# david-andrew/TerminalRayTracer

Hardware: AMD Instinct MI355X
Metric: path rays/s (primary+secondary) at 1920x1080, 64 spheres, 8 bounces (higher is better)
Workload: dtype f64

## Files before the change

include/trt_hip_diag.h:

```cpp
#ifndef TRT_HIP_DIAG_H
#define TRT_HIP_DIAG_H

#include "trt_hip.h"

#ifdef __cplusplus
extern "C" {
#endif

int trt_set_list_pool_words(trt_context *ctx, size_t words);

int trt_enable_counters(trt_context *ctx, int enable);

int trt_read_counters(trt_context *ctx, unsigned long long *path_rays, unsigned long long *shadow_rays);

int trt_read_diagnostics(trt_context *ctx, unsigned long long *wave_loop_trips, unsigned long long *phase2_rounds);

int trt_path_family_code(trt_context *ctx, int kind, int sphere, const double *parent_origin);

long trt_read_path_tables(trt_context *ctx, const Camera *camera, unsigned long long *cells, size_t capacity_cells,
                          unsigned long long *pool, size_t capacity_pool, long info[8]);

int trt_read_sweep_fallbacks(trt_context *ctx, unsigned long long *swept_traces);

int trt_read_shading_passes(trt_context *ctx, unsigned long long *passes);

int trt_read_loop_diagnostics(trt_context *ctx, unsigned long long out[8]);

long trt_read_light_grid(trt_context *ctx, int point_light, int index, unsigned long long *masks, size_t capacity_words);

long trt_read_light_lists(trt_context *ctx, int point_light, int index, unsigned long long *cells, size_t capacity_cells,
                          unsigned long long *pool, size_t capacity_pool, long info[4]);

int trt_selftest_div_sqrt(trt_context *ctx, const double *a, const double *b, size_t n, double *quot, double *root);

int trt_selftest_unit(trt_context *ctx, const double *xyzw, size_t n, double *fast, double *reference);

int trt_selftest_cube(trt_context *ctx, const float *xyz, size_t n, float *device_out, float *host_out);

int trt_selftest_sky(trt_context *ctx, const double *dirs, size_t n, int dim, long long *exact, long long *estimate, int *ambiguous);

int trt_probe_rays(trt_context *ctx, const Ray *rays, size_t n, int *obj, double *point, double *normal,
                   double *material, double *lit);

int trt_probe_rays_production(trt_context *ctx, const Camera *camera, const Ray *rays, const int *families, size_t n, int *obj,
                              double *point, double *normal, double *material, double *lit);

long trt_launch_count(trt_context *ctx);
int trt_launch_span_ms(trt_context *first, long first_launch, trt_context *last, long last_launch, float *ms);

int trt_set_scene_image(trt_context *ctx, int mode);

int trt_render_image(trt_context *ctx, int *in_device_memory, unsigned long long *image_bytes);

// ... 16 lines not shown
```

terminalraytracer_amd/csrc/trt_context.hpp:

```cpp
#pragma once

#include "trt_hip.h"
#include "trt_hip_diag.h"

#include <hip/hip_runtime.h>

#include <math.h>
#include <stdarg.h>
#include <stdio.h>
#include <stdlib.h>
#include <string.h>

#include <algorithm>
#include <chrono>
#include <memory>
#include <mutex>
#include <thread>
#include <vector>

#ifndef TRT_DIRGRID_CELLS
#define TRT_DIRGRID_CELLS 128
#endif
#ifndef TRT_POINTGRID_CELLS
#define TRT_POINTGRID_CELLS 64
// ... 57 lines not shown
    double m = fmod(t, 2 * kPi);
    return (m < kPi) ? (m / kPi) : (2 - (m / kPi));
}

}

using trt_impl::DeviceBuffer;
using trt_impl::Event;
using trt_impl::PinnedBuffer;
using trt_impl::Stream;
using trt_impl::kEventRing;

constexpr int kEyeSlots = 8;

struct SceneTables
{
    int device = 0;
    DeviceBuffer<double> d_spheres, d_dir, d_point;
    DeviceBuffer<float> d_cull;
    DeviceBuffer<unsigned long long> d_dir_masks, d_point_masks;
    DeviceBuffer<trt_dirgrid> d_dirgrids;
    DeviceBuffer<trt_pointgrid> d_pointgrids;
    DeviceBuffer<trt_dirgrid_disc> d_discs;
    DeviceBuffer<trt_pointgrid_cone> d_cones;
    DeviceBuffer<unsigned long long> d_dir_lists, d_point_lists, d_path_lists, d_pool;
    DeviceBuffer<unsigned long long> d_pool_used;
    DeviceBuffer<trt_rayfamily> d_families;
    DeviceBuffer<double> d_sphere_fam;
    DeviceBuffer<double> d_patch_rec;
    DeviceBuffer<uint32_t> d_sky;
    int path_built_for[4] = {-1, -1, -1, -2};
    int grids_built_for[4] = {-1, -1, -1, -1};
    size_t pool_scene_words = 0, pool_eye_words = 0;
    trt_cull_scene cull_scene{};
    double ground_built[6] = {0.0, 0.0, 0.0, 0.0, 0.0, 0.0};
    std::vector<double> h_spheres, h_dir, h_point;
    unsigned eye_slots_taken = 0;
    bool built_for_moving_scene = false;
    double build_seconds = 0.0;
    ~SceneTables() { (void)hipSetDevice(device); }
};

struct trt_context
{
    int device = 0;
    Stream own_stream;
    hipStream_t stream = nullptr;
    int compute_units = 0;
    int reserved_cus = 0;
    int lds_limit = 0;

    bool have_scene = false;
    std::shared_ptr<SceneTables> T;
    int eye_slot = 0;
    trt::SceneView scene{};
    trt::CullView cull{};
    DeviceBuffer<double> d_jitter, d_fb, d_axes, d_samples, d_samples_alt;
    DeviceBuffer<double> d_image, d_image_alt;
    trt::GridView grids{};
    int dirgrid_cells = TRT_DIRGRID_CELLS, pointgrid_cells = TRT_POINTGRID_CELLS;
    int dirgrid_slabs = TRT_DIRGRID_SLABS, pointgrid_shells = TRT_POINTGRID_SHELLS;
    int path_g_eye = TRT_PATHGRID_EYE, path_g_sph = TRT_PATHGRID_SPHERE;
    int path_min_spheres = TRT_PATHGRID_MIN_SPHERES;
    int path_patches = TRT_PATHGRID_PATCHES;
    size_t list_pool_cap = 0;
    int scene_changes_in_a_row = 0, scene_still_calls = 0;
// ... 139 lines not shown
```

terminalraytracer_amd/csrc/trt_diag.hip:

```cpp
#define TRT_UNIT_DIAG 1
#include "trt_context.hpp"
#include "trt_simple.hpp"

using namespace trt_impl;

namespace trt_impl
{
void allow_large_lds_diag(const trt_context *ctx)
{
    (void)hipFuncSetAttribute((const void *)trt::probe_rays_kernel, hipFuncAttributeMaxDynamicSharedMemorySize, ctx->lds_limit);
    (void)hipFuncSetAttribute((const void *)trt::probe_rounds_kernel<false>, hipFuncAttributeMaxDynamicSharedMemorySize, ctx->lds_limit);
    (void)hipFuncSetAttribute((const void *)trt::probe_rounds_kernel<true>, hipFuncAttributeMaxDynamicSharedMemorySize, ctx->lds_limit);
}
}

extern "C" int trt_set_list_pool_words(trt_context *ctx, size_t words)
{
    if (!ctx)
        return fail(TRT_ERR_ARGUMENT, "ctx is NULL");
    const int rc = refuse_if_shared(ctx, "trt_set_list_pool_words");
    if (rc)
        return rc;
    ctx->list_pool_cap = words;
    ctx->T->grids_built_for[0] = -1;
// ... 54 lines not shown
    const int k = trt_patch_of(ctx->grids.patch_m, parent_origin[0] - c[0], parent_origin[1] - c[1], parent_origin[2] - c[2]);
    return 2 + n + ((sphere << TRT_PATCH_SHIFT) | k);
}

extern "C" long trt_read_path_tables(trt_context *ctx, const Camera *camera, unsigned long long *cells, size_t capacity_cells,
                                     unsigned long long *pool, size_t capacity_pool, long info[8])
{
    if (!ctx || !camera || !cells || !pool || !info)
        return fail(TRT_ERR_ARGUMENT, "NULL argument");
    if (!ctx->have_scene)
        return fail(TRT_ERR_NO_SCENE, "no scene");
    HIP_TRY(hipSetDevice(ctx->device));
    const int rc = ensure_eye_tables(ctx, camera, ctx->stream);
    if (rc)
        return rc;
    HIP_TRY(hipStreamSynchronize(ctx->stream));
    const trt::GridView &g = ctx->grids;
    const int n = (int)(ctx->T->h_spheres.size() / 9);
    unsigned long long used[16 * (1 + kEyeSlots)] = {0};
    HIP_TRY(hipMemcpy(used, ctx->T->d_pool_used.ptr, sizeof used, hipMemcpyDeviceToHost));
    const size_t eye_total = 2 * 6 * (size_t)g.g_eye * g.g_eye, sph_total = 2 * (size_t)n * (size_t)g.patch_count * 6 * (size_t)g.g_sph * g.g_sph;
    const size_t total = g.path_enabled ? eye_total + sph_total : 0;
    const size_t pool_words = ctx->T->pool_scene_words + kEyeSlots * ctx->T->pool_eye_words;
    const size_t eye_from = ctx->T->pool_scene_words + (size_t)ctx->eye_slot * ctx->T->pool_eye_words;
    info[0] = g.path_enabled, info[1] = g.g_eye, info[2] = g.g_sph, info[3] = n, info[4] = (long)total;
    info[5] = (long)std::min<unsigned long long>(used[0], 1ull << 62), info[6] = (long)used[16 * (1 + ctx->eye_slot)] - (long)eye_from, info[7] = (long)pool_words;
    if (!g.path_enabled)
        return 0;
    if (capacity_cells < total || capacity_pool < pool_words)
        return fail(TRT_ERR_CAPACITY, "tables have %zu cells and %zu pool words", total, pool_words);
    HIP_TRY(hipMemcpy(cells, ctx->T->d_path_lists.ptr + g.eye_at, eye_total * sizeof(unsigned long long), hipMemcpyDeviceToHost));
    if (sph_total)
        HIP_TRY(hipMemcpy(cells + eye_total, ctx->T->d_path_lists.ptr + g.sph_at, sph_total * sizeof(unsigned long long), hipMemcpyDeviceToHost));
    HIP_TRY(hipMemcpy(pool, ctx->T->d_pool.ptr, pool_words * sizeof(unsigned long long), hipMemcpyDeviceToHost));
    return (long)total;
}

extern "C" long trt_read_light_grid(trt_context *ctx, int point_light, int index, unsigned long long *masks, size_t capacity_words)
{
    if (!ctx || !masks || index < 0)
        return fail(TRT_ERR_ARGUMENT, "bad argument");
    if (!ctx->have_scene)
        return fail(TRT_ERR_NO_SCENE, "no scene");
    const trt::GridView &g = ctx->grids;
    if (!g.enabled)
        return 0;
    if (index >= (point_light ? ctx->scene.num_point : ctx->scene.num_dir))
        return fail(TRT_ERR_ARGUMENT, "light %d", index);
    const size_t words = (size_t)std::max((ctx->scene.num_spheres + 63) / 64, 1);
    const size_t stride = (point_light ? g.point_stride : g.dir_stride) * words;
    if (capacity_words < stride)
        return fail(TRT_ERR_CAPACITY, "table has %zu words, buffer %zu", stride, capacity_words);
    HIP_TRY(hipSetDevice(ctx->device));
    HIP_TRY(hipStreamSynchronize(ctx->stream));
    HIP_TRY(hipMemcpy(masks, (point_light ? ctx->T->d_point_masks.ptr : ctx->T->d_dir_masks.ptr) + stride * (size_t)index, stride * sizeof(unsigned long long),
                      hipMemcpyDeviceToHost));
    return (long)stride;
}

extern "C" long trt_read_light_lists(trt_context *ctx, int point_light, int index, unsigned long long *cells, size_t capacity_cells,
                                     unsigned long long *pool, size_t capacity_pool, long info[4])
{
    const bool query = !cells && !pool && !capacity_cells && !capacity_pool;
    if (!ctx || !info || index < 0 || (!query && (!cells || !pool)))
        return fail(TRT_ERR_ARGUMENT, "bad argument");
    if (!ctx->have_scene)
// ... 223 lines not shown
```

terminalraytracer_amd/csrc/trt_rounds.hpp:

```cpp
#pragma once

#include "trt_device.hpp"
#include "trt_filter.h"
#include "trt_lightgrid.h"
#include "trt_raygrid.h"
#include "trt_common.hpp"

#define TRT_EXPECT_LIST(c) __builtin_expect(!!(c), 1)
#define TRT_EXPECT_RARE(c) __builtin_expect(!!(c), 0)

namespace trt
{


#define CONSTANT_AS __attribute__((address_space(4)))
template <class T>
TRT_DEV T load_kernel_argument(const char CONSTANT_AS *at)
{
    static_assert(sizeof(T) % 8 == 0 && alignof(T) == 8, "argument structs are whole 64-bit words");
    T out;
    const unsigned long long CONSTANT_AS *src = (const unsigned long long CONSTANT_AS *)at;
    unsigned long long *dst = (unsigned long long *)&out;
#pragma unroll
    for (size_t i = 0; i < sizeof(T) / 8; i++)
        dst[i] = src[i];
    return out;
}

struct GridView
{
    const trt_dirgrid *dir;
    const trt_pointgrid *point;
    const unsigned long long *dir_lists, *point_lists;
    unsigned dir_stride, point_stride;
    int enabled;
    int list_bits;
    int path_enabled;
    int g_eye, g_sph;
    int patch_m, patch_count;
    unsigned eye_at, sph_at;
    const unsigned long long *path_lists;
    const unsigned long long *pool;
    const double *sphere_fam;
    const double *patch_rec;
    double rg2_sph;
    double slack0;
    trt_rayfamily eye[2];
};

static_assert(sizeof(trt_rayfamily) == 8 * TRT_RAYFAMILY_DOUBLES, "families of the eye in the LDS image");
static_assert(sizeof(trt_dirgrid) == 8 * kDirGridDoubles && sizeof(trt_pointgrid) == 8 * kPointGridDoubles, "light-table headers in the LDS image");

constexpr int kDirRecord = 8;

struct LdsImage
{
    const float4 *cull;
    const float4 *cull_dir;
    const double *sph;
    const double *mat;
    const double *dir;
    const double *pt;
    const double *b255;
    const double *cam;
    const double *jit;
    const trt_dirgrid *dirgrid;
    const trt_pointgrid *pointgrid;
    const double *fam;
    const double *eye;
    const double *patch;
};

inline size_t rounds_lds_bytes(const SceneView &s, int spp, int patches, int frames = 1)
// ... 373 lines not shown
        k++;
        const double2 c01 = ((const double2 *)L.sph)[2 * i], c23 = ((const double2 *)L.sph)[2 * i + 1];
        const d3 oc = sub(o, d3{c01.x, c01.y, c23.x});
        const double b = 2.0 * dot(oc, d);
        const double cc = dot(oc, oc) - c23.y;
        const double disc = b * b - 4.0 * a * cc;
        if (valid && !(disc < 0.0) && b < 0.0)
        {
            const double q = -b - sqrt_exact(disc), qq = q * q;
            const bool blocks = q > TRT_SHADOW_QMIN && qq * TRT_SHADOW_K1 <= lo;
            unsure = unsure || (q > 0.0 && !blocks && !(qq >= hi));
            dark = dark || blocks;
            count = blocks ? 0 : count;
        }
    }
    {
        const double denom = dot(d, gn), num = dot(sub(gp, o), gn);
        const bool steep = __builtin_fabs(denom) > 0.00001;
        const bool same_sign = (long long)(__builtin_bit_cast(unsigned long long, num) ^ __builtin_bit_cast(unsigned long long, denom)) >= 0;
        const bool maybe = active && !dark && steep && same_sign;
        if (__any(maybe))
        {
            const double t = num / denom;
            const bool hit = maybe && t > 0.00001;
            const double qq = (t * t) * (4.0 * a) * a;
            const bool blocks = hit && qq * TRT_SHADOW_K1 <= lo;
            dark = dark || blocks;
            unsure = unsure || (hit && !blocks && !(qq >= hi));
        }
    }
    unsure = unsure && !dark;
}

template <bool BATCH = false>
TRT_DEV unsigned long long path_cell(const LdsImage &L, const GridView &G, int n, int fam, d3 o, d3 d, bool active, unsigned long long active_lanes,
                                     unsigned long long &fallback_lanes, int frame = 0)
{
    const bool in_family = fam >= 0;
    const unsigned long long family_lanes = lanes_with(in_family);
    const bool has = active && in_family;
    const int f = has ? fam : 0;
    const int s = f >= 2 ? f - 2 : 0, i = s >= n ? s - n : s;
    const bool of_eye = f < 2, mirrored = s >= n;
    const double *rec = L.fam + 4 * i;
    d3 apex = mirrored ? load3(rec) : load3(L.sph + 4 * i);
    double r_chk = mirrored ? rec[3] + TRT_FAMILY_SLACK : rec[3];
    const double *E = BATCH ? L.eye + frame * (2 * TRT_RAYFAMILY_DOUBLES) + TRT_RAYFAMILY_DOUBLES * (f & 1) : L.eye + TRT_RAYFAMILY_DOUBLES * (f & 1);
    const double rg2_eye = E[5];
    if (of_eye)
    {
        apex = load3(E);
        r_chk = E[3];
    }
    const double rg2 = of_eye ? rg2_eye : G.rg2_sph;
    const d3 w = sub(o, apex);
    const d3 c = d3{w.y * d.z - w.z * d.y, w.z * d.x - w.x * d.z, w.x * d.y - w.y * d.x};
    const bool near_line = dot(c, c) <= r_chk * r_chk, ahead = dot(w, d) >= -r_chk, in_range = dot(w, w) <= rg2;
    const bool unit_dir = __builtin_fabs(dot(d, d) - 1.0) <= 9.094947017729282e-13;
    const bool member = near_line & ahead & in_range & unit_dir;
    const unsigned long long member_lanes = family_lanes & lanes_with(near_line) & lanes_with(ahead) & lanes_with(in_range) & lanes_with(unit_dir);
    const int g = of_eye ? G.g_eye : G.g_sph;
    const int at = trt_cubemap_cell((float)d.x, (float)d.y, (float)d.z, 0.5f * (float)g, (float)(g - 1), g);
    const unsigned eye_cells = 6u * (unsigned)G.g_eye * (unsigned)G.g_eye, sph_cells = 6u * (unsigned)G.g_sph * (unsigned)G.g_sph;
    const unsigned base = of_eye ? G.eye_at + (BATCH ? 2u * (unsigned)frame + (unsigned)f : (unsigned)f) * eye_cells : G.sph_at + (unsigned)s * sph_cells;
    unsigned long long cell = 0;
    if (has && member)
        cell = G.path_lists[base + (unsigned)at];
    fallback_lanes = active_lanes & (~member_lanes | lanes_with((unsigned)(cell >> 56) == TRT_LIST_NONE));
    return cell;
}

template <bool BATCH = false>
TRT_DEV unsigned long long path_cell_patches(const LdsImage &L, const GridView &G, int n, int &fam, d3 o, d3 d, bool active, unsigned long long active_lanes,
                                             unsigned long long &fallback_lanes, int frame = 0)
{
    const bool in_family = fam >= 0;
    const unsigned long long family_lanes = lanes_with(in_family);
    const bool has = active && in_family;
    const int f = has ? fam : 0;
    const bool of_eye = f < 2, mirrored = f >= 2 + n;
    const int code = f - 2 - n;
    const int i = mirrored ? code >> TRT_PATCH_SHIFT : (of_eye ? 0 : f - 2);
    const double *at_sphere = L.sph + 4 * i, *at_mirror = L.fam + 4 * i;
    const double *src = of_eye ? L.eye + (BATCH ? frame * (2 * TRT_RAYFAMILY_DOUBLES) : 0) + TRT_RAYFAMILY_DOUBLES * (f & 1) : (mirrored ? at_mirror : at_sphere);
    const d3 base_at = load3(src);
    const int here = trt_cubemap_cell((float)(o.x - base_at.x), (float)(o.y - base_at.y), (float)(o.z - base_at.z), 0.5f * (float)G.patch_m,
                                      (float)(G.patch_m - 1), G.patch_m);
    const int k = mirrored ? code & ((1 << TRT_PATCH_SHIFT) - 1) : (of_eye ? 0 : here);
    fam = !has ? -1 : (f == 0 ? 1 : (!of_eye && !mirrored ? 2 + n + (((f - 2) << TRT_PATCH_SHIFT) | k) : -1));
    const double r_abs = of_eye ? 0.0 : at_mirror[3];
    const double *pr = L.patch + TRT_PATCH_RECORD * k + (mirrored ? 4 : 0);
    const d3 apex = d3{TRT_PATCH_APEX(base_at.x, r_abs, pr[0]), TRT_PATCH_APEX(base_at.y, r_abs, pr[1]), TRT_PATCH_APEX(base_at.z, r_abs, pr[2])};
    const double rho = pr[3];
    double rchk_eye = src[3], rg2_eye = src[5];
    asm("" : "+v"(rchk_eye), "+v"(rg2_eye));
    double r_chk = TRT_PATCH_RCHK(r_abs, rho, G.slack0), rg2 = G.rg2_sph;
    r_chk = mirrored ? r_chk + TRT_FAMILY_SLACK : r_chk;
// ... 23 lines not shown
}

struct Tally
{
    unsigned path = 0, shadow = 0, rounds = 0, swept = 0, passes = 0;
    unsigned iters[3] = {0, 0, 0};
    unsigned tests[3] = {0, 0, 0};
    unsigned full = 0;
};

struct PathHit
{
    Hit ph;
    bool hit;
    bool sky;
    unsigned long long hit_lanes, sky_lanes;
    d3 back;
    d3 normal;
    int mat;
};

template <bool COUNT, bool REFRACT = false, bool PATCHES = false, bool BATCH = false>
TRT_DEV PathHit path_stage(const LdsImage &L, const CullView &cull, const GridView &grids, int n, d3 o, d3 d, int &fam, bool alive, unsigned long long alive_lanes,
                           d3 gp, d3 gn, Tally &tally, int inside = -1, int frame = 0)
{
    bool p_list = false;
    unsigned long long p_cell = 0;
    if (grids.path_enabled)
    {
        unsigned long long fallback_lanes;
        if constexpr (PATCHES)
            p_cell = path_cell_patches<BATCH>(L, grids, n, fam, o, d, alive, alive_lanes, fallback_lanes, frame);
        else
            p_cell = path_cell<BATCH>(L, grids, n, fam, o, d, alive, alive_lanes, fallback_lanes, frame);
        p_list = fallback_lanes == 0;
    }
    if (COUNT && !p_list)
        tally.swept++;
    PathHit r;
    r.ph = trace<false, REFRACT, 2>(L, cull, n, o, d, alive, alive_lanes, gp, gn, tally.iters[0], tally.tests[0], nullptr, p_list, p_cell, grids.pool, grids.list_bits, inside);
    r.hit = alive && r.ph.i >= 0;
    r.sky = alive && r.ph.i < 0;
    r.hit_lanes = alive_lanes & lanes_with(r.ph.i >= 0);
    r.sky_lanes = alive_lanes & ~r.hit_lanes;
    if (r.hit)
        fam = r.ph.i < n ? 2 + r.ph.i : (PATCHES ? fam : (fam == 0 ? 1 : (fam >= 2 && fam < 2 + n ? fam + n : -1)));
    r.back = unit(r.hit ? sub(o, r.ph.p) : d);
    r.normal = d;
    r.mat = 0;
    if (r.hit_lanes != 0)
    {
        d3 raw = gn;
        r.mat = n + checker_odd(r.ph.p);
        if (r.ph.i >= 0 && r.ph.i < n)
        {
            raw = sub(r.ph.p, load3(L.sph + 4 * r.ph.i));
            r.mat = r.ph.i;
        }
        r.normal = unit(raw);
    }
    TRT_MARK_AT(6);
    return r;
}

template <bool COUNT>
TRT_DEV d3 shadow_stage(const LdsImage &L, const CullView &cull, const GridView &grids, int n, int nd, int nl, d3 o, d3 normal, int mat,
                        bool lit_lanes, unsigned long long lit_word, d3 gp, d3 gn, Tally &tally)
// ... 669 lines not shown
```

terminalraytracer_amd/csrc/trt_tables.hip:

```cpp
#include "trt_context.hpp"

using namespace trt_impl;

namespace
{

__global__ void build_dirgrid_kernel(const trt_dirgrid_disc *discs, int n, int g, int slabs, int words, unsigned long long *masks)
{
    const long cell = (long)blockIdx.x * blockDim.x + threadIdx.x;
    if (cell >= (long)slabs * g * g)
        return;
    const int c = (int)(cell % g), j = (int)((cell / g) % g), slab = (int)(cell / ((long)g * g));
    for (int w = 0; w < words; w++)
    {
        unsigned long long m = 0;
        for (int b = 0; b < 64 && w * 64 + b < n; b++)
            if (trt_dirgrid_in_slab(discs + w * 64 + b, slab) && trt_dirgrid_reaches(discs + w * 64 + b, c, j))
                m |= 0x8000000000000000ull >> b;
        masks[cell * words + w] = m;
    }
}

__global__ void build_pointgrid_kernel(const trt_pointgrid_cone *cones, int n, int g, int shells, int words, unsigned long long *masks)
{
// ... 10 lines not shown
        masks[cell * words + w] = m;
    }
}

__device__ unsigned long long pack_cell(const unsigned long long *mask, int words, unsigned long long *pool, unsigned long long *pool_used,
                                        unsigned pool_limit, int bits, bool valid = true)
{
    const int count = valid ? trt_list_count(mask, words) : 0;
    const unsigned need = valid ? trt_list_pool_words(count, bits) : 0u;
    const int lane = (int)(threadIdx.x & 63);
    unsigned upto = need;
#pragma unroll
    for (int d = 1; d < 64; d <<= 1)
    {
        const unsigned below = __shfl_up(upto, d);
        upto += lane >= d ? below : 0u;
    }
    const unsigned total = __shfl(upto, 63);
    unsigned long long base = 0;
    if (total)
    {
        if (lane == 63)
            base = atomicAdd(pool_used, (unsigned long long)total);
        base = __shfl(base, 63);
    }
    if (!valid)
        return 0ull;
    if (need == 0)
        return trt_list_pack(mask, words, count, nullptr, 0u, bits);
    const unsigned long long at = base + (upto - need);
    if (count > 0xffff || at + need > (unsigned long long)pool_limit)
        return (unsigned long long)TRT_LIST_NONE << 56;
    return trt_list_pack(mask, words, count, pool, (unsigned)at, bits);
}

__global__ void set_pool_counter_kernel(unsigned long long *counter, unsigned long long value) { *counter = value; }

__global__ void pack_lists_kernel(const unsigned long long *masks, long cells, int words, unsigned long long *lists, unsigned long long *pool,
                                  unsigned long long *pool_used, unsigned pool_limit, int bits)
{
    const long cell = (long)blockIdx.x * blockDim.x + threadIdx.x;
    const bool valid = cell < cells;
    const unsigned long long packed = pack_cell(masks + (valid ? cell : 0) * words, words, pool, pool_used, pool_limit, bits, valid);
    if (valid)
        lists[cell] = packed;
}

static_assert(TRT_FAMILY_TILE * TRT_FAMILY_TILE == 64, "a tile per wave");
constexpr int kSceneTilesPerBlock = 16;
unsigned family_grid_blocks(int g, int tiles_per_block)
{
    const unsigned cells = 6u * (unsigned)g * (unsigned)g;
    return trt_family_tiled(g) ? (cells / 64u + (unsigned)tiles_per_block - 1u) / (unsigned)tiles_per_block : (cells + 255u) / 256u;
}

template <int kWords>
constexpr size_t family_lds_bytes()
{
    return sizeof(trt_pointgrid_cone) * 64 * kWords + sizeof(unsigned long long) * kWords + sizeof(unsigned long long) * 4 * 64 * kWords;
}

template <int kWords>
__global__ __launch_bounds__(256) void build_family_lists_kernel(const double *spheres, int n, const trt_rayfamily *families, trt_rayfamily f0,
                                                                 trt_rayfamily f1, int by_value, int g, unsigned long long *lists,
                                                                 unsigned long long *pool, unsigned long long *pool_used, unsigned pool_limit,
                                                                 int tiles_per_block)
// ... 175 lines not shown
{
    if (ctx->path_patches >= 0)
        return std::min(ctx->path_patches, TRT_PATCH_MAX_M);
    if (ctx->moving_scene)
        return 0;
    int m = n >= TRT_PATCHES_FROM_SPHERES ? 2 : 0;
    const unsigned long long per_table = 6ull * (unsigned long long)ctx->path_g_sph * (unsigned long long)ctx->path_g_sph;
    while (m > 0 && 2ull * (unsigned long long)n * (6ull * m * m) * per_table * 12ull > kAutoPatchBudgetBytes)
        m--;
    return m;
}

static int build_path_tables(trt_context *ctx, const trt_cull_scene &cs, const double *ground)
{
    const int n = (int)(ctx->T->h_spheres.size() / 9);
    trt::GridView &g = ctx->grids;
    g.path_enabled = 0;
    g.patch_m = g.patch_count = 0;
    invalidate_eye_tables(ctx);
    ctx->T->path_built_for[0] = ctx->path_g_eye;
    ctx->T->path_built_for[1] = ctx->path_g_sph;
    ctx->T->path_built_for[2] = ctx->path_min_spheres;
    ctx->T->path_built_for[3] = ctx->path_patches;
    ctx->T->cull_scene = cs;
    memcpy(ctx->T->ground_built, ground, sizeof ctx->T->ground_built);
    const int ge = ctx->path_g_eye, gs = ctx->path_g_sph;
    if (ge < 2 || gs < 2 || n > TRT_PATH_MAX_SPHERES || n < ctx->path_min_spheres)
        return TRT_OK;
    trt_patchset patches;
    trt_patchset_init(&patches, patches_for(ctx, n));
    const size_t P = (size_t)patches.count, families = 2 * (size_t)n * P;
    const size_t eye_cells = 6 * (size_t)ge * ge, sph_cells = 6 * (size_t)gs * gs;
    const size_t eye_part = (size_t)kEyeSlots * 2 * eye_cells;
    if (eye_part + families * sph_cells >= 0xffffffffull)
        return fail(TRT_ERR_CAPACITY, "path tables of %zu families x %zu cells", families, sph_cells);
    HIP_TRY(ctx->T->d_path_lists.reserve(eye_part + families * sph_cells));
    HIP_TRY(hipMemsetAsync(ctx->T->d_path_lists.ptr, 0xFF, (eye_part + families * sph_cells) * sizeof(unsigned long long), ctx->stream));
    HIP_TRY(ctx->T->d_families.reserve(std::max<size_t>(families, 1)));
    HIP_TRY(ctx->T->d_sphere_fam.reserve(4 * (size_t)std::max(n, 1)));
    HIP_TRY(ctx->T->d_patch_rec.reserve(P * TRT_PATCH_RECORD));
    std::vector<trt_rayfamily> fam(std::max<size_t>(families, 1));
    std::vector<double> rec(4 * (size_t)std::max(n, 1)), prec(P * TRT_PATCH_RECORD);
    trt_family_consts consts;
    trt_sphere_families(ctx->T->h_spheres.data(), n, ground, &cs, &patches, fam.data(), rec.data(), &consts);
    trt_patch_records(&patches, ground, prec.data());
    HIP_TRY(hipMemcpy(ctx->T->d_patch_rec.ptr, prec.data(), prec.size() * sizeof(double), hipMemcpyHostToDevice));
    if (n)
    {
        HIP_TRY(hipMemcpy(ctx->T->d_families.ptr, fam.data(), families * sizeof(trt_rayfamily), hipMemcpyHostToDevice));
        HIP_TRY(hipMemcpy(ctx->T->d_sphere_fam.ptr, rec.data(), 4 * (size_t)n * sizeof(double), hipMemcpyHostToDevice));
        for (size_t first = 0; first < families; first += 32768)
        {
            const unsigned batch = (unsigned)std::min<size_t>(32768, families - first);
            launch_family_builder(n, dim3(family_grid_blocks(gs, kSceneTilesPerBlock), batch), ctx->stream, (const double *)ctx->T->d_spheres.ptr,
                                  (const trt_rayfamily *)ctx->T->d_families.ptr + first, trt_rayfamily{}, trt_rayfamily{}, 0, gs,
                                  ctx->T->d_path_lists.ptr + eye_part + first * sph_cells, ctx->T->d_pool.ptr, ctx->T->d_pool_used.ptr, (unsigned)ctx->T->pool_scene_words,
                                  kSceneTilesPerBlock);
        }
        HIP_TRY(hipGetLastError());
        HIP_TRY(hipStreamSynchronize(ctx->stream));
    }
    g.path_lists = ctx->T->d_path_lists.ptr;
    g.eye_at = (unsigned)((size_t)ctx->eye_slot * 2 * eye_cells);
    g.sph_at = (unsigned)eye_part;
    g.pool = ctx->T->d_pool.ptr;
    g.sphere_fam = ctx->T->d_sphere_fam.ptr;
    g.patch_rec = ctx->T->d_patch_rec.ptr;
    g.patch_m = patches.m;
    g.patch_count = patches.count;
    g.rg2_sph = consts.rg * consts.rg;
    g.slack0 = consts.slack;
    g.g_eye = ge;
    g.g_sph = gs;
    g.path_enabled = 1;
    return TRT_OK;
}

int build_tables(trt_context *ctx, const trt_cull_scene &cs, const double *ground)
{
    ctx->table_builds++;
    const size_t n = ctx->T->h_spheres.size() / 9, nd = ctx->T->h_dir.size() / 6, np = ctx->T->h_point.size() / 7;
    const size_t gd = (size_t)ctx->dirgrid_cells, gp = (size_t)ctx->pointgrid_cells, ge = (size_t)ctx->path_g_eye, gs = (size_t)ctx->path_g_sph;
    const size_t sd = (size_t)std::max(ctx->dirgrid_slabs, 1), sp = (size_t)std::max(ctx->pointgrid_shells, 1);
    const int m = patches_for(ctx, (int)n);
    const size_t sphere_cells = 2 * n * (m ? 6 * (size_t)m * m : 1) * 6 * gs * gs;
    const size_t wide = n > TRT_LIST_MAX_SPHERES ? 2 : 1, sphere_part = n > TRT_PATH_MAX_SPHERES ? 0 : (m ? sphere_cells / 2 : sphere_cells);
    ctx->T->pool_scene_words = std::max<size_t>(1024, wide * (nd * sd * gd * gd + np * 6 * sp * gp * gp + sphere_part));
    const size_t per_word = wide == 2 ? 4 : 8;
    ctx->T->pool_eye_words = std::max<size_t>(1024, 2 * 6 * ge * ge * std::min<size_t>((n + per_word - 1) / per_word, 64));
    if (ctx->list_pool_cap)
    {
        ctx->T->pool_scene_words = std::min(ctx->T->pool_scene_words, std::max<size_t>(ctx->list_pool_cap, 1));
        ctx->T->pool_eye_words = std::min(ctx->T->pool_eye_words, std::max<size_t>(ctx->list_pool_cap, 1));
    }
    const double t0 = host_seconds();
    int rc = TRT_OK;
    for (int pass = 0; pass < 2 && !rc; pass++)
    {
        if (ctx->T->pool_scene_words + kEyeSlots * ctx->T->pool_eye_words >= 0xffffffffull)
            return fail(TRT_ERR_CAPACITY, "candidate tables too large");
        ctx->grids = trt::GridView{};
        ctx->grids.list_bits = n > TRT_LIST_MAX_SPHERES ? 16 : 8;
        HIP_TRY(ctx->T->d_pool.reserve(ctx->T->pool_scene_words + kEyeSlots * ctx->T->pool_eye_words));
        HIP_TRY(ctx->T->d_pool_used.reserve(16 * (1 + kEyeSlots)));
        HIP_TRY(hipMemsetAsync(ctx->T->d_pool_used.ptr, 0, 16 * (1 + kEyeSlots) * sizeof(unsigned long long), ctx->stream));
        rc = build_light_grids(ctx, cs);
        if (!rc)
            rc = build_path_tables(ctx, cs, ground);
        if (rc || ctx->list_pool_cap)
            break;
        unsigned long long asked = 0;
        HIP_TRY(hipMemcpyAsync(&asked, ctx->T->d_pool_used.ptr, sizeof asked, hipMemcpyDeviceToHost, ctx->stream));
        HIP_TRY(hipStreamSynchronize(ctx->stream));
        if (asked <= ctx->T->pool_scene_words)
            break;
        ctx->T->pool_scene_words = (size_t)asked + 1024;
    }
    ctx->T->build_seconds = host_seconds() - t0;
    return rc;
}

static int build_eye_slot(trt_context *ctx, const trt_rayfamily *families, int slot, hipStream_t stream)
{
    const trt::GridView &g = ctx->grids;
    const int n = (int)(ctx->T->h_spheres.size() / 9), ge = g.g_eye;
    const size_t eye_cells = 6 * (size_t)ge * ge;
    const size_t pool_from = ctx->T->pool_scene_words + (size_t)slot * ctx->T->pool_eye_words;
    unsigned long long *const counter = ctx->T->d_pool_used.ptr + 16 * (1 + slot);
    hipLaunchKernelGGL(set_pool_counter_kernel, dim3(1), dim3(1), 0, stream, counter, (unsigned long long)pool_from);
    launch_family_builder(n, dim3(family_grid_blocks(ge, 1), 2u), stream, (const double *)ctx->T->d_spheres.ptr, (const trt_rayfamily *)nullptr, families[0], families[1], 1,
                          ge, ctx->T->d_path_lists.ptr + (size_t)slot * 2 * eye_cells, ctx->T->d_pool.ptr, counter, (unsigned)(pool_from + ctx->T->pool_eye_words), 1);
    HIP_TRY(hipGetLastError());
    return TRT_OK;
}

int ensure_eye_tables(trt_context *ctx, const Camera *camera, hipStream_t stream, int slot)
{
    trt::GridView &g = ctx->grids;
    if (!g.path_enabled)
        return TRT_OK;
    if (slot < 0)
        slot = ctx->eye_slot;
    trt_context::EyeSlot &built = ctx->eye_slots[slot];
    const double eye[3] = {camera->frame.origin.x, camera->frame.origin.y, camera->frame.origin.z};
    if (built.valid && !memcmp(eye, built.eye, sizeof eye))
        return TRT_OK;
    built.valid = false;
    trt_eye_families(eye, ctx->T->ground_built, &ctx->T->cull_scene, built.families);
    if (slot == ctx->eye_slot)
// ... 11 lines not shown
```

terminalraytracer_amd/hip.py:

```python
import ctypes as C
import functools
import os

import numpy as np

from . import layout as L

_HERE = os.path.dirname(os.path.abspath(__file__))
LIB_PATH = os.environ.get("TRT_HIP_LIB") or os.path.join(_HERE, "libtrt_hip.so")

TRT_OK = 0
ERRORS = {-1: "TRT_ERR_HIP", -2: "TRT_ERR_ARGUMENT", -3: "TRT_ERR_NO_SCENE", -4: "TRT_ERR_CAPACITY",
          -5: "TRT_ERR_NOT_INITIALISED"}


class TrtError(RuntimeError):
    def __init__(self, code, message):
        super().__init__(f"{ERRORS.get(code, code)}: {message}")
        self.code = code


class RowSet(C.Structure):
    _fields_ = [("width", C.c_int), ("height", C.c_int), ("tile_rows", C.c_int), ("tile_first", C.c_int),
                ("tile_step", C.c_int)]
# ... 51 lines not shown
    "trt_render_host_batch": (_I, [_VP, _VP, _I, C.POINTER(RowSet), _I, _I, _VP]),
    "trt_render_device_batch_rgb8": (_I, [_VP, _VP, _I, C.POINTER(RowSet), _I, _I, _VP, _SZ]),
    "trt_render_host_batch_rgb8": (_I, [_VP, _VP, _I, C.POINTER(RowSet), _I, _I, _VP]),
    "trt_render_device_batch_ansi": (_I, [_VP, _VP, _I, C.POINTER(RowSet), _I, _I, _VP, _SZ]),
    "trt_render_host_batch_ansi": (_I, [_VP, _VP, _I, C.POINTER(RowSet), _I, _I, _VP]),
    "trt_batch_info": (_I, [_VP, C.POINTER(_I), C.POINTER(_I)]),
    "trt_synchronize": (_I, [_VP]),
    "trt_kernel_times": (_I, [_VP, C.POINTER(C.c_float), _I]),
    "trt_render_kernel_times": (_I, [_VP, C.POINTER(C.c_float), C.POINTER(C.c_float), _I]),
    "trt_enable_counters": (_I, [_VP, _I]),
    "trt_read_counters": (_I, [_VP, C.POINTER(C.c_ulonglong), C.POINTER(C.c_ulonglong)]),
    "trt_read_diagnostics": (_I, [_VP, C.POINTER(C.c_ulonglong), C.POINTER(C.c_ulonglong)]),
    "trt_set_kernel": (_I, [_VP, _I]),
    "trt_set_light_grids": (_I, [_VP, _I, _I]),
    "trt_set_light_slabs": (_I, [_VP, _I, _I]),
    "trt_share_scene": (_I, [_VP, _VP]),
    "trt_set_scene_policy": (_I, [_I, _I]),
    "trt_scene_is_moving": (_I, []),
    "trt_scene_info": (_I, [_VP, C.POINTER(C.c_ulonglong), C.POINTER(_I), C.POINTER(C.c_double)]),
    "trt_set_list_pool_words": (_I, [_VP, C.c_size_t]),
    "trt_set_path_grids": (_I, [_VP, _I, _I]),
    "trt_set_path_grids_min_spheres": (_I, [_VP, _I]),
    "trt_set_path_patches": (_I, [_VP, _I]),
    "trt_get_path_patches": (_I, [_VP, C.POINTER(_I), C.POINTER(_I)]),
    "trt_path_family_code": (_I, [_VP, _I, _I, _VP]),
    "trt_set_compaction": (_I, [_VP, _I]),
    "trt_render_variant": (_I, [_VP, C.POINTER(_I), C.POINTER(_I)]),
    "trt_set_scene_image": (_I, [_VP, _I]),
    "trt_render_image": (_I, [_VP, C.POINTER(_I), C.POINTER(C.c_ulonglong)]),
    "trt_set_scratch_fill": (_I, [_VP, _I]),
    "trt_default_context": (_VP, []),
    "trt_build_counts": (_I, [_VP, C.POINTER(C.c_ulonglong), C.POINTER(C.c_ulonglong)]),
    "trt_read_path_tables": (C.c_long, [_VP, C.POINTER(L.Camera), _VP, C.c_size_t, _VP, C.c_size_t, C.POINTER(C.c_long)]),
    "trt_read_sweep_fallbacks": (_I, [_VP, C.POINTER(C.c_ulonglong)]),
    "trt_read_shading_passes": (_I, [_VP, C.POINTER(C.c_ulonglong)]),
    "trt_read_loop_diagnostics": (_I, [_VP, C.POINTER(C.c_ulonglong)]),
    "trt_set_refraction": (_I, [_VP, _VP, _I]),
    "trt_reserve_cus": (_I, [_VP, _I]),
    "trt_get_stream": (_I, [_VP, C.POINTER(C.c_void_p)]),
    "trt_selftest_cube": (_I, [_VP, _VP, C.c_size_t, _VP, _VP]),
    "trt_selftest_unit": (_I, [_VP, _VP, C.c_size_t, _VP, _VP]),
    "trt_selftest_sky": (_I, [_VP, _VP, C.c_size_t, _I, _VP, _VP, _VP]),
    "trt_read_light_grid": (C.c_long, [_VP, _I, _I, _VP, C.c_size_t]),
    "trt_read_light_lists": (C.c_long, [_VP, _I, _I, _VP, C.c_size_t, _VP, C.c_size_t, C.POINTER(C.c_long)]),
    "trt_kernel_info": (_I, [_VP] + [C.POINTER(_I)] * 5),
    "trt_selftest_div_sqrt": (_I, [_VP, _VP, _VP, _SZ, _VP, _VP]),
    "trt_probe_rays": (_I, [_VP, _VP, _SZ, _VP, _VP, _VP, _VP, _VP]),
    "trt_probe_rays_production": (_I, [_VP, C.POINTER(L.Camera), _VP, _VP, _SZ, _VP, _VP, _VP, _VP, _VP]),
    "trt_launch_count": (C.c_long, [_VP]),
    "trt_launch_span_ms": (_I, [_VP, C.c_long, _VP, C.c_long, C.POINTER(C.c_float)]),
    "trt_dist_unique_id": (_I, [_VP]),
    "trt_dist_frame_times": (_I, [_VP, C.POINTER(C.c_float), C.POINTER(C.c_float)]),
    "trt_dist_allow_rccl_override": (_I, [_I]),
    "trt_dist_rccl_library": (C.c_char_p, []),
    "trt_dist_comm_ranks": (_I, [_VP]),
    "trt_dist_create": (_I, [_I, C.POINTER(L.Scene), _VP, _I, _I, _I, _I, _I, _I, _I, C.POINTER(_VP)]),
    "trt_dist_set_scene": (_I, [_VP, C.POINTER(L.Scene)]),
    "trt_dist_render": (_I, [_VP, C.POINTER(L.Camera), _I, _I, C.POINTER(_VP)]),
    "trt_dist_synchronize": (_I, [_VP]),
    "trt_dist_enable_rgb8": (_I, [_VP]),
    "trt_dist_render_rgb8": (_I, [_VP, C.POINTER(L.Camera), _I, _I, C.POINTER(_VP)]),
    "trt_dist_fetch_rgb8": (_I, [_VP, _VP, _VP]),
    "trt_dist_fetch": (_I, [_VP, _VP, _VP]),
    "trt_dist_source_rows": (_I, [_I, _I, _I, _I, C.POINTER(_I)]),
    "trt_dist_info": (_I, [_VP] + [C.POINTER(_I)] * 5),
    "trt_dist_context": (_VP, [_VP, _I]),
# ... 131 lines not shown
        d, t = _I(), _I()
        _check(lib().trt_render_variant(self._h, C.byref(d), C.byref(t)))
        return {"decoupled": bool(d.value), "workgroup_threads": t.value}

    def set_scene_image(self, mode):
        _check(lib().trt_set_scene_image(self._h, mode))

    def render_image(self):
        d, b = _I(), C.c_ulonglong()
        _check(lib().trt_render_image(self._h, C.byref(d), C.byref(b)))
        return {"in_device_memory": bool(d.value), "image_bytes": b.value}

    def build_counts(self):
        b, u = C.c_ulonglong(), C.c_ulonglong()
        _check(lib().trt_build_counts(self._h, C.byref(b), C.byref(u)))
        return b.value, u.value

    def set_scratch_fill(self, on=True):
        _check(lib().trt_set_scratch_fill(self._h, 1 if on else 0))

    def read_path_tables(self, camera_array):
        cam = camera_struct(camera_array)
        info = (C.c_long * 8)()
        probe = np.zeros(1, dtype=np.uint64)
        lib().trt_read_path_tables(self._h, C.byref(cam), probe.ctypes.data, 0, probe.ctypes.data, 0, info)
        cells = np.zeros(max(1, info[4]), dtype=np.uint64)
        pool = np.zeros(max(1, info[7]), dtype=np.uint64)
        got = lib().trt_read_path_tables(self._h, C.byref(cam), cells.ctypes.data, cells.size, pool.ctypes.data, pool.size, info)
        if got < 0:
            _check(int(got))
        keys = ("enabled", "eye_cells", "sphere_cells", "spheres", "cells", "pool_used_scene", "pool_used_eye", "pool_capacity")
        return dict(zip(keys, [int(x) for x in info])), cells[:got], pool

    def set_refraction(self, ior=None):
        if ior is None:
            _check(lib().trt_set_refraction(self._h, None, 0))
        else:
            a = np.ascontiguousarray(ior, dtype=np.float64)
            _check(lib().trt_set_refraction(self._h, a.ctypes.data, a.size))

    def read_sweep_fallbacks(self):
        v = C.c_ulonglong()
        _check(lib().trt_read_sweep_fallbacks(self._h, C.byref(v)))
        return v.value

    def selftest_unit(self, xyzw):
        v = np.ascontiguousarray(xyzw, dtype=np.float64).reshape(-1, 4)
        fast, ref = np.zeros_like(v), np.zeros_like(v)
        _check(lib().trt_selftest_unit(self._h, v.ctypes.data, v.shape[0], fast.ctypes.data, ref.ctypes.data))
        return fast, ref

    def selftest_cube(self, xyz):
        v = np.ascontiguousarray(xyz, dtype=np.float32).reshape(-1, 3)
        dev, host = np.zeros((v.shape[0], 4), dtype=np.float32), np.zeros((v.shape[0], 4), dtype=np.float32)
        _check(lib().trt_selftest_cube(self._h, v.ctypes.data, v.shape[0], dev.ctypes.data, host.ctypes.data))
        return dev, host

    def selftest_sky(self, dirs, dim):
        v = np.ascontiguousarray(dirs, dtype=np.float64).reshape(-1, 3)
        exact, est = np.zeros(v.shape[0], dtype=np.int64), np.zeros(v.shape[0], dtype=np.int64)
        amb = np.zeros(v.shape[0], dtype=np.int32)
        _check(lib().trt_selftest_sky(self._h, v.ctypes.data, v.shape[0], int(dim), exact.ctypes.data, est.ctypes.data, amb.ctypes.data))
        return exact, est, amb

    def read_light_grid(self, point_light, index, words):
        out = np.zeros(words, dtype=np.uint64)
# ... 408 lines not shown
```

Before: 37.38 billion.

## Add per-sphere candidate lists with the emitting sphere stripped for outgoing rays

Builds an extra set of per-sphere path candidate lists at table-build time, removing each sphere's own index from its lists, and stores them in a separate pool region. At trace time, non-refractive rays leaving a sphere surface (positive along-direction) look up the stripped table, so the self-intersection test against the emitting sphere is no longer done. This costs more table memory, an extra build kernel and a third pool-resize pass, and adds a diagnostic reader for the new tables.

```diff
diff --git a/include/trt_hip_diag.h b/include/trt_hip_diag.h
--- a/include/trt_hip_diag.h
+++ b/include/trt_hip_diag.h
@@ -19,6 +19,9 @@
 
 long trt_read_path_tables(trt_context *ctx, const Camera *camera, unsigned long long *cells, size_t capacity_cells,
                           unsigned long long *pool, size_t capacity_pool, long info[8]);
+
+long trt_read_own_tables(trt_context *ctx, unsigned long long *cells, size_t capacity_cells, unsigned long long *pool, size_t capacity_pool,
+                         long info[8]);
 
 int trt_read_sweep_fallbacks(trt_context *ctx, unsigned long long *swept_traces);
 
diff --git a/terminalraytracer_amd/csrc/trt_context.hpp b/terminalraytracer_amd/csrc/trt_context.hpp
--- a/terminalraytracer_amd/csrc/trt_context.hpp
+++ b/terminalraytracer_amd/csrc/trt_context.hpp
@@ -113,6 +113,7 @@
     int path_built_for[4] = {-1, -1, -1, -2};
     int grids_built_for[4] = {-1, -1, -1, -1};
     size_t pool_scene_words = 0, pool_eye_words = 0;
+    size_t pool_own_words = 0, own_cells = 0;
     trt_cull_scene cull_scene{};
     double ground_built[6] = {0.0, 0.0, 0.0, 0.0, 0.0, 0.0};
     std::vector<double> h_spheres, h_dir, h_point;
diff --git a/terminalraytracer_amd/csrc/trt_diag.hip b/terminalraytracer_amd/csrc/trt_diag.hip
--- a/terminalraytracer_amd/csrc/trt_diag.hip
+++ b/terminalraytracer_amd/csrc/trt_diag.hip
@@ -110,6 +110,34 @@
     HIP_TRY(hipMemcpy(cells, ctx->T->d_path_lists.ptr + g.eye_at, eye_total * sizeof(unsigned long long), hipMemcpyDeviceToHost));
     if (sph_total)
         HIP_TRY(hipMemcpy(cells + eye_total, ctx->T->d_path_lists.ptr + g.sph_at, sph_total * sizeof(unsigned long long), hipMemcpyDeviceToHost));
+    HIP_TRY(hipMemcpy(pool, ctx->T->d_pool.ptr, pool_words * sizeof(unsigned long long), hipMemcpyDeviceToHost));
+    return (long)total;
+}
+
+extern "C" long trt_read_own_tables(trt_context *ctx, unsigned long long *cells, size_t capacity_cells, unsigned long long *pool, size_t capacity_pool,
+                                    long info[8])
+{
+    const bool query = !cells && !pool && !capacity_cells && !capacity_pool;
+    if (!ctx || !info || (!query && (!cells || !pool)))
+        return fail(TRT_ERR_ARGUMENT, "bad argument");
+    if (!ctx->have_scene)
+        return fail(TRT_ERR_NO_SCENE, "no scene");
+    HIP_TRY(hipSetDevice(ctx->device));
+    HIP_TRY(hipStreamSynchronize(ctx->stream));
+    const trt::GridView &g = ctx->grids;
+    const int n = (int)(ctx->T->h_spheres.size() / 9);
+    const size_t total = g.path_enabled ? ctx->T->own_cells : 0;
+    const size_t own_from = ctx->T->pool_scene_words + kEyeSlots * ctx->T->pool_eye_words, pool_words = own_from + ctx->T->pool_own_words;
+    unsigned long long upto = 0;
+    if (total)
+        HIP_TRY(hipMemcpy(&upto, ctx->T->d_pool_used.ptr + 16 * (1 + kEyeSlots), sizeof upto, hipMemcpyDeviceToHost));
+    info[0] = total != 0, info[1] = g.g_sph, info[2] = n, info[3] = (long)total, info[4] = total ? (long)(upto - own_from) : 0, info[5] = (long)own_from;
+    info[6] = (long)pool_words, info[7] = g.list_bits;
+    if (!total || query)
+        return (long)total;
+    if (capacity_cells < total || capacity_pool < pool_words)
+        return fail(TRT_ERR_CAPACITY, "tables have %zu cells and %zu pool words", total, pool_words);
+    HIP_TRY(hipMemcpy(cells, ctx->T->d_path_lists.ptr + g.own_at, total * sizeof(unsigned long long), hipMemcpyDeviceToHost));
     HIP_TRY(hipMemcpy(pool, ctx->T->d_pool.ptr, pool_words * sizeof(unsigned long long), hipMemcpyDeviceToHost));
     return (long)total;
 }
diff --git a/terminalraytracer_amd/csrc/trt_ownlist.h b/terminalraytracer_amd/csrc/trt_ownlist.h
--- /dev/null
+++ b/terminalraytracer_amd/csrc/trt_ownlist.h
@@ -0,0 +1,55 @@
+#ifndef TRT_OWNLIST_H
+#define TRT_OWNLIST_H
+
+#include "trt_raygrid.h"
+
+TRT_HD int trt_list_strip_count(unsigned long long cell, const unsigned long long *pool, int own, int bits)
+{
+    const int e = trt_list_entries(cell);
+    int kept = 0;
+    for (int k = 0; k < e; k++)
+        kept += trt_list_entry(cell, pool, k, bits) != own;
+    return e < 0 ? -1 : kept;
+}
+
+TRT_HD unsigned long long trt_list_strip(unsigned long long cell, const unsigned long long *pool, int own, int bits, int kept,
+                                         unsigned long long *out_pool, unsigned out_at)
+{
+    const int per = 64 / bits, inline_max = 56 / bits;
+    const int e = trt_list_entries(cell);
+    if (e < 0 || kept < 0)
+        return (unsigned long long)TRT_LIST_NONE << 56;
+    if (kept <= inline_max)
+    {
+        unsigned long long out = (unsigned long long)kept << 56;
+        int j = 0;
+        for (int k = 0; k < e; k++)
+        {
+            const int i = trt_list_entry(cell, pool, k, bits);
+            if (i != own)
+                out |= (unsigned long long)(unsigned)i << (bits * j++);
+        }
+        return out;
+    }
+    if (!out_pool)
+        return (unsigned long long)TRT_LIST_NONE << 56;
+    unsigned long long cur = 0;
+    int j = 0;
+    for (int k = 0; k < e; k++)
+    {
+        const int i = trt_list_entry(cell, pool, k, bits);
+        if (i == own)
+            continue;
+        cur |= (unsigned long long)(unsigned)i << (bits * (j % per));
+        if (++j % per == 0)
+        {
+            out_pool[out_at + (unsigned)(j / per) - 1u] = cur;
+            cur = 0;
+        }
+    }
+    if (j % per)
+        out_pool[out_at + (unsigned)(j / per)] = cur;
+    return ((unsigned long long)TRT_LIST_POOLED << 56) | ((unsigned long long)(unsigned)kept << 32) | out_at;
+}
+
+#endif
diff --git a/terminalraytracer_amd/csrc/trt_rounds.hpp b/terminalraytracer_amd/csrc/trt_rounds.hpp
--- a/terminalraytracer_amd/csrc/trt_rounds.hpp
+++ b/terminalraytracer_amd/csrc/trt_rounds.hpp
@@ -4,6 +4,7 @@
 #include "trt_filter.h"
 #include "trt_lightgrid.h"
 #include "trt_raygrid.h"
+#include "trt_ownlist.h"
 #include "trt_common.hpp"
 
 #define TRT_EXPECT_LIST(c) __builtin_expect(!!(c), 1)
@@ -39,6 +40,7 @@
     int g_eye, g_sph;
     int patch_m, patch_count;
     unsigned eye_at, sph_at;
+    unsigned own_at;
     const unsigned long long *path_lists;
     const unsigned long long *pool;
     const double *sphere_fam;
@@ -478,7 +480,7 @@
     unsure = unsure && !dark;
 }
 
-template <bool BATCH = false>
+template <bool BATCH = false, bool STRIPPED = true>
 TRT_DEV unsigned long long path_cell(const LdsImage &L, const GridView &G, int n, int fam, d3 o, d3 d, bool active, unsigned long long active_lanes,
                                      unsigned long long &fallback_lanes, int frame = 0)
 {
@@ -501,14 +503,19 @@
     const double rg2 = of_eye ? rg2_eye : G.rg2_sph;
     const d3 w = sub(o, apex);
     const d3 c = d3{w.y * d.z - w.z * d.y, w.z * d.x - w.x * d.z, w.x * d.y - w.y * d.x};
-    const bool near_line = dot(c, c) <= r_chk * r_chk, ahead = dot(w, d) >= -r_chk, in_range = dot(w, w) <= rg2;
+    const double along = dot(w, d);
+    const bool near_line = dot(c, c) <= r_chk * r_chk, ahead = along >= -r_chk, in_range = dot(w, w) <= rg2;
     const bool unit_dir = __builtin_fabs(dot(d, d) - 1.0) <= 9.094947017729282e-13;
     const bool member = near_line & ahead & in_range & unit_dir;
     const unsigned long long member_lanes = family_lanes & lanes_with(near_line) & lanes_with(ahead) & lanes_with(in_range) & lanes_with(unit_dir);
+    const bool leaves_own = STRIPPED && (unsigned)(f - 2) < (unsigned)n && along >= 0.0;
     const int g = of_eye ? G.g_eye : G.g_sph;
     const int at = trt_cubemap_cell((float)d.x, (float)d.y, (float)d.z, 0.5f * (float)g, (float)(g - 1), g);
     const unsigned eye_cells = 6u * (unsigned)G.g_eye * (unsigned)G.g_eye, sph_cells = 6u * (unsigned)G.g_sph * (unsigned)G.g_sph;
-    const unsigned base = of_eye ? G.eye_at + (BATCH ? 2u * (unsigned)frame + (unsigned)f : (unsigned)f) * eye_cells : G.sph_at + (unsigned)s * sph_cells;
+    unsigned own_at = G.own_at, sph_at = G.sph_at;
+    asm("" : "+s"(own_at), "+s"(sph_at));
+    const unsigned sph_from = leaves_own ? own_at : sph_at;
+    const unsigned base = of_eye ? G.eye_at + (BATCH ? 2u * (unsigned)frame + (unsigned)f : (unsigned)f) * eye_cells : sph_from + (unsigned)s * sph_cells;
     unsigned long long cell = 0;
     if (has && member)
         cell = G.path_lists[base + (unsigned)at];
@@ -598,7 +605,7 @@
         if constexpr (PATCHES)
             p_cell = path_cell_patches<BATCH>(L, grids, n, fam, o, d, alive, alive_lanes, fallback_lanes, frame);
         else
-            p_cell = path_cell<BATCH>(L, grids, n, fam, o, d, alive, alive_lanes, fallback_lanes, frame);
+            p_cell = path_cell<BATCH, !REFRACT>(L, grids, n, fam, o, d, alive, alive_lanes, fallback_lanes, frame);
         p_list = fallback_lanes == 0;
     }
     if (COUNT && !p_list)
diff --git a/terminalraytracer_amd/csrc/trt_tables.hip b/terminalraytracer_amd/csrc/trt_tables.hip
--- a/terminalraytracer_amd/csrc/trt_tables.hip
+++ b/terminalraytracer_amd/csrc/trt_tables.hip
@@ -66,6 +66,38 @@
     if (count > 0xffff || at + need > (unsigned long long)pool_limit)
         return (unsigned long long)TRT_LIST_NONE << 56;
     return trt_list_pack(mask, words, count, pool, (unsigned)at, bits);
+}
+
+__global__ void strip_own_lists_kernel(const unsigned long long *full, unsigned long long *stripped, unsigned cells, unsigned sph_cells,
+                                       unsigned long long *pool, unsigned long long *pool_used, unsigned pool_limit, int bits)
+{
+    const unsigned cell = blockIdx.x * blockDim.x + threadIdx.x;
+    const bool valid = cell < cells;
+    const unsigned long long in = valid ? full[cell] : (unsigned long long)TRT_LIST_NONE << 56;
+    const int own = (int)(cell / sph_cells);
+    const int kept = trt_list_strip_count(in, pool, own, bits);
+    const unsigned need = kept > 0 ? trt_list_pool_words(kept, bits) : 0u;
+    const int lane = (int)(threadIdx.x & 63);
+    unsigned upto = need;
+#pragma unroll
+    for (int d = 1; d < 64; d <<= 1)
+    {
+        const unsigned below = __shfl_up(upto, d);
+        upto += lane >= d ? below : 0u;
+    }
+    const unsigned total = __shfl(upto, 63);
+    unsigned long long base = 0;
+    if (total)
+    {
+        if (lane == 63)
+            base = atomicAdd(pool_used, (unsigned long long)total);
+        base = __shfl(base, 63);
+    }
+    if (!valid)
+        return;
+    const unsigned long long at = base + (upto - need);
+    const bool room = at + need <= (unsigned long long)pool_limit;
+    stripped[cell] = trt_list_strip(in, pool, own, bits, kept, room ? pool : nullptr, (unsigned)at);
 }
 
 __global__ void set_pool_counter_kernel(unsigned long long *counter, unsigned long long value) { *counter = value; }
@@ -307,10 +339,12 @@
     const size_t P = (size_t)patches.count, families = 2 * (size_t)n * P;
     const size_t eye_cells = 6 * (size_t)ge * ge, sph_cells = 6 * (size_t)gs * gs;
     const size_t eye_part = (size_t)kEyeSlots * 2 * eye_cells;
-    if (eye_part + families * sph_cells >= 0xffffffffull)
+    const size_t own_cells = patches.m == 0 ? (size_t)n * sph_cells : 0;
+    ctx->T->own_cells = own_cells;
+    if (eye_part + families * sph_cells + own_cells >= 0xffffffffull)
         return fail(TRT_ERR_CAPACITY, "path tables of %zu families x %zu cells", families, sph_cells);
-    HIP_TRY(ctx->T->d_path_lists.reserve(eye_part + families * sph_cells));
-    HIP_TRY(hipMemsetAsync(ctx->T->d_path_lists.ptr, 0xFF, (eye_part + families * sph_cells) * sizeof(unsigned long long), ctx->stream));
+    HIP_TRY(ctx->T->d_path_lists.reserve(eye_part + families * sph_cells + own_cells));
+    HIP_TRY(hipMemsetAsync(ctx->T->d_path_lists.ptr, 0xFF, (eye_part + families * sph_cells + own_cells) * sizeof(unsigned long long), ctx->stream));
     HIP_TRY(ctx->T->d_families.reserve(std::max<size_t>(families, 1)));
     HIP_TRY(ctx->T->d_sphere_fam.reserve(4 * (size_t)std::max(n, 1)));
     HIP_TRY(ctx->T->d_patch_rec.reserve(P * TRT_PATCH_RECORD));
@@ -332,12 +366,22 @@
                                   ctx->T->d_path_lists.ptr + eye_part + first * sph_cells, ctx->T->d_pool.ptr, ctx->T->d_pool_used.ptr, (unsigned)ctx->T->pool_scene_words,
                                   kSceneTilesPerBlock);
         }
+        if (own_cells)
+        {
+            const size_t own_from = ctx->T->pool_scene_words + kEyeSlots * ctx->T->pool_eye_words;
+            unsigned long long *const counter = ctx->T->d_pool_used.ptr + 16 * (1 + kEyeSlots);
+            hipLaunchKernelGGL(set_pool_counter_kernel, dim3(1), dim3(1), 0, ctx->stream, counter, (unsigned long long)own_from);
+            hipLaunchKernelGGL(strip_own_lists_kernel, dim3((unsigned)((own_cells + 255) / 256)), dim3(256), 0, ctx->stream,
+                               (const unsigned long long *)(ctx->T->d_path_lists.ptr + eye_part), ctx->T->d_path_lists.ptr + eye_part + families * sph_cells,
+                               (unsigned)own_cells, (unsigned)sph_cells, ctx->T->d_pool.ptr, counter, (unsigned)(own_from + ctx->T->pool_own_words), g.list_bits);
+        }
         HIP_TRY(hipGetLastError());
         HIP_TRY(hipStreamSynchronize(ctx->stream));
     }
     g.path_lists = ctx->T->d_path_lists.ptr;
     g.eye_at = (unsigned)((size_t)ctx->eye_slot * 2 * eye_cells);
     g.sph_at = (unsigned)eye_part;
+    g.own_at = own_cells ? (unsigned)(eye_part + families * sph_cells) : g.sph_at;
     g.pool = ctx->T->d_pool.ptr;
     g.sphere_fam = ctx->T->d_sphere_fam.ptr;
     g.patch_rec = ctx->T->d_patch_rec.ptr;
@@ -363,33 +407,42 @@
     ctx->T->pool_scene_words = std::max<size_t>(1024, wide * (nd * sd * gd * gd + np * 6 * sp * gp * gp + sphere_part));
     const size_t per_word = wide == 2 ? 4 : 8;
     ctx->T->pool_eye_words = std::max<size_t>(1024, 2 * 6 * ge * ge * std::min<size_t>((n + per_word - 1) / per_word, 64));
+    ctx->T->pool_own_words = m == 0 && n > 0 && n <= TRT_PATH_MAX_SPHERES && (int)n >= ctx->path_min_spheres && ge >= 2 && gs >= 2 ? std::max<size_t>(1024, wide * n * 6 * gs * gs) : 0;
     if (ctx->list_pool_cap)
     {
         ctx->T->pool_scene_words = std::min(ctx->T->pool_scene_words, std::max<size_t>(ctx->list_pool_cap, 1));
         ctx->T->pool_eye_words = std::min(ctx->T->pool_eye_words, std::max<size_t>(ctx->list_pool_cap, 1));
+        ctx->T->pool_own_words = std::min(ctx->T->pool_own_words, std::max<size_t>(ctx->list_pool_cap, 1));
     }
     const double t0 = host_seconds();
     int rc = TRT_OK;
-    for (int pass = 0; pass < 2 && !rc; pass++)
-    {
-        if (ctx->T->pool_scene_words + kEyeSlots * ctx->T->pool_eye_words >= 0xffffffffull)
+    for (int pass = 0; pass < 3 && !rc; pass++)
+    {
+        const size_t pool_words = ctx->T->pool_scene_words + kEyeSlots * ctx->T->pool_eye_words + ctx->T->pool_own_words;
+        if (pool_words >= 0xffffffffull)
             return fail(TRT_ERR_CAPACITY, "candidate tables too large");
         ctx->grids = trt::GridView{};
         ctx->grids.list_bits = n > TRT_LIST_MAX_SPHERES ? 16 : 8;
-        HIP_TRY(ctx->T->d_pool.reserve(ctx->T->pool_scene_words + kEyeSlots * ctx->T->pool_eye_words));
-        HIP_TRY(ctx->T->d_pool_used.reserve(16 * (1 + kEyeSlots)));
-        HIP_TRY(hipMemsetAsync(ctx->T->d_pool_used.ptr, 0, 16 * (1 + kEyeSlots) * sizeof(unsigned long long), ctx->stream));
+        HIP_TRY(ctx->T->d_pool.reserve(pool_words));
+        HIP_TRY(ctx->T->d_pool_used.reserve(16 * (2 + kEyeSlots)));
+        HIP_TRY(hipMemsetAsync(ctx->T->d_pool_used.ptr, 0, 16 * (2 + kEyeSlots) * sizeof(unsigned long long), ctx->stream));
         rc = build_light_grids(ctx, cs);
         if (!rc)
             rc = build_path_tables(ctx, cs, ground);
         if (rc || ctx->list_pool_cap)
             break;
-        unsigned long long asked = 0;
+        unsigned long long asked = 0, own_upto = 0;
         HIP_TRY(hipMemcpyAsync(&asked, ctx->T->d_pool_used.ptr, sizeof asked, hipMemcpyDeviceToHost, ctx->stream));
+        HIP_TRY(hipMemcpyAsync(&own_upto, ctx->T->d_pool_used.ptr + 16 * (1 + kEyeSlots), sizeof own_upto, hipMemcpyDeviceToHost, ctx->stream));
         HIP_TRY(hipStreamSynchronize(ctx->stream));
-        if (asked <= ctx->T->pool_scene_words)
+        const size_t own_from = ctx->T->pool_scene_words + kEyeSlots * ctx->T->pool_eye_words;
+        const unsigned long long own_asked = own_upto > own_from ? own_upto - own_from : 0;
+        if (asked <= ctx->T->pool_scene_words && own_asked <= ctx->T->pool_own_words)
             break;
-        ctx->T->pool_scene_words = (size_t)asked + 1024;
+        if (asked > ctx->T->pool_scene_words)
+            ctx->T->pool_scene_words = (size_t)asked + 1024;
+        if (own_asked > ctx->T->pool_own_words)
+            ctx->T->pool_own_words = (size_t)own_asked + 1024;
     }
     ctx->T->build_seconds = host_seconds() - t0;
     return rc;
diff --git a/terminalraytracer_amd/hip.py b/terminalraytracer_amd/hip.py
--- a/terminalraytracer_amd/hip.py
+++ b/terminalraytracer_amd/hip.py
@@ -107,6 +107,7 @@
     "trt_default_context": (_VP, []),
     "trt_build_counts": (_I, [_VP, C.POINTER(C.c_ulonglong), C.POINTER(C.c_ulonglong)]),
     "trt_read_path_tables": (C.c_long, [_VP, C.POINTER(L.Camera), _VP, C.c_size_t, _VP, C.c_size_t, C.POINTER(C.c_long)]),
+    "trt_read_own_tables": (C.c_long, [_VP, _VP, C.c_size_t, _VP, C.c_size_t, C.POINTER(C.c_long)]),
     "trt_read_sweep_fallbacks": (_I, [_VP, C.POINTER(C.c_ulonglong)]),
     "trt_read_shading_passes": (_I, [_VP, C.POINTER(C.c_ulonglong)]),
     "trt_read_loop_diagnostics": (_I, [_VP, C.POINTER(C.c_ulonglong)]),
@@ -304,6 +305,20 @@
         keys = ("enabled", "eye_cells", "sphere_cells", "spheres", "cells", "pool_used_scene", "pool_used_eye", "pool_capacity")
         return dict(zip(keys, [int(x) for x in info])), cells[:got], pool
 
+    def read_own_tables(self):
+        info = (C.c_long * 8)()
+        got = lib().trt_read_own_tables(self._h, None, 0, None, 0, info)
+        if got < 0:
+            _check(int(got))
+        cells = np.zeros(max(1, info[3]), dtype=np.uint64)
+        pool = np.zeros(max(1, info[6]), dtype=np.uint64)
+        if got:
+            got = lib().trt_read_own_tables(self._h, cells.ctypes.data, cells.size, pool.ctypes.data, pool.size, info)
+            if got < 0:
+                _check(int(got))
+        keys = ("enabled", "sphere_cells", "spheres", "cells", "pool_used", "pool_from", "pool_capacity", "list_bits")
+        return dict(zip(keys, [int(x) for x in info])), cells[:got], pool
+
     def set_refraction(self, ior=None):
         if ior is None:
             _check(lib().trt_set_refraction(self._h, None, 0))
```

Result: no change. 37.74 billion (median of 6 runs) (+1.0%).
